# NVIDIA/makani

Measured on NVIDIA H100. Metric: SFNO-block fwd+bwd samples/sec, higher is better.
Workload: dtype tf32

## Files before the change

makani_b200/csrc/dft.cu:

```cuda
#include "umma_common.cuh"
#include "dft_math.cuh"
#include <cmath>
#include <cstdlib>
#include <vector>

namespace b200sht {

int umma_available();

constexpr int kDftMaxHalf = 95;
constexpr int kDftSynWorkers = 10;
constexpr int kDftSynThreads = 32 * (kDftSynWorkers + 2);
constexpr int kDftSynStages = 4;
__host__ __device__ constexpr int dft_out_box(int N2) {
  int d = N2 < 32 ? N2 : 32;
  while (N2 % d != 0) --d;
  return 8 * d;
}

struct DftTables {
  float* et;
  float* eb;
  float2* tw;
  float* zeros;
  int N2, half, M2, nkb;
};

bool dft_shape_ok(int nlon, int mmax) {
  if (nlon % 8 != 0) return false;
  const int N2 = nlon / 8;
  return N2 >= 2 && N2 / 2 <= kDftMaxHalf && (mmax + 7) / 8 <= 32 && mmax <= nlon / 2 + 1;
}

__global__ void dft_tables_kernel(float* et, float* eb, float2* tw, int N2, int half, int M2, int nkb, int nlon) {
  const int i = blockIdx.x * blockDim.x + threadIdx.x;
  if (i < 2 * 128 * 32) {
    const int m2 = i % 32, row = i / 32, p = (row >> 3) & 1, j2 = 8 * (row >> 4) + (row & 7);
    float v = 0.f;
    if (j2 <= half && m2 < M2) {
      const long long t = ((long long)m2 * j2) % N2;
      const double ang = 2.0 * M_PI * (double)t / (double)N2;
      v = tf32_rn((float)(p == 0 ? cos(ang) : sin(ang)));
    }
    et[i] = v;
  }
  if (i < nkb * 2 * 32 * 32) {
    const int jl = i % 32, m2 = (i / 32) % 32, p = (i / 1024) % 2, kb = i / 2048;
    const int j2 = kb * 32 + jl;
    float v = 0.f;
    if (j2 <= half && m2 < M2) {
      const long long t = ((long long)m2 * j2) % N2;
      const double ang = 2.0 * M_PI * (double)t / (double)N2;
      v = tf32_rn((float)(p == 0 ? cos(ang) : sin(ang)));
      if (2 * j2 == N2) v *= 0.5f;
    }
    eb[i] = v;
  }
  if (i < 8 * N2) {
    const int j2 = i % N2, c = i / N2;
    const double ang = 2.0 * M_PI * (double)(c * j2) / (double)nlon;
    tw[i] = make_float2((float)cos(ang), (float)sin(ang));
  }
}

int dft_plan_init(Plan* pl) {
  pl->dft_state = nullptr;
  if (!umma_available()) return -1;
  if (!dft_shape_ok(pl->nlon, pl->mmax)) return -1;
  DftTables* t = new DftTables();
  t->N2 = pl->nlon / 8; t->half = t->N2 / 2; t->M2 = (pl->mmax + 7) / 8;
  t->nkb = (t->half + 1 + 31) / 32;
  t->et = nullptr; t->eb = nullptr; t->tw = nullptr; t->zeros = nullptr;
  const size_t neb = (size_t)t->nkb * 2 * 32 * 32;
  cudaError_t e = cudaMalloc(&t->et, sizeof(float) * 2 * 128 * 32);
  if (e == cudaSuccess) e = cudaMalloc(&t->eb, sizeof(float) * neb);
  if (e == cudaSuccess) e = cudaMalloc(&t->tw, sizeof(float2) * 8 * t->N2);
  if (e == cudaSuccess) e = cudaMalloc(&t->zeros, sizeof(float) * 8 * t->N2);
  if (e == cudaSuccess) e = cudaMemset(t->zeros, 0, sizeof(float) * 8 * t->N2);
  if (e == cudaSuccess) {
    const int n = 8192 > 8 * t->N2 ? 8192 : 8 * t->N2;
    dft_tables_kernel<<<(n + 255) / 256, 256>>>(t->et, t->eb, t->tw, t->N2, t->half, t->M2, t->nkb, pl->nlon);
    e = cudaGetLastError();
    if (e == cudaSuccess) e = cudaStreamSynchronize(0);
  }
  if (e != cudaSuccess) {
    cudaFree(t->et); cudaFree(t->eb); cudaFree(t->tw); cudaFree(t->zeros);
    delete t;
    return -1;
  }
  pl->dft_state = t;
  return 0;
}

void dft_plan_destroy(Plan* pl) {
  DftTables* t = static_cast<DftTables*>(pl->dft_state);
  if (!t) return;
  cudaFree(t->et); cudaFree(t->eb); cudaFree(t->tw); cudaFree(t->zeros);
  delete t;
  pl->dft_state = nullptr;
}

static bool dft_enabled() {
  static const int on = [] { const char* e = getenv("B200SHT_DFT"); return e ? atoi(e) : 1; }();
  return on != 0;
}
bool dft_usable(const Plan* pl) { return pl->dft_state != nullptr && dft_enabled(); }

static unsigned long long* g_dft_prof = nullptr;
static unsigned long long* dft_prof_buffer() {
  static const int on = [] { const char* e = getenv("B200SHT_DFT_PROF"); return e ? atoi(e) : 0; }();
  if (!on) return nullptr;
  if (!g_dft_prof) {
    if (cudaMalloc(&g_dft_prof, 16 * sizeof(unsigned long long)) != cudaSuccess) { g_dft_prof = nullptr; return nullptr; }
    cudaMemset(g_dft_prof, 0, 16 * sizeof(unsigned long long));
  }
  return g_dft_prof;
}
int dft_profile_read(unsigned long long* out16) {
  if (!g_dft_prof) { for (int i = 0; i < 16; ++i) out16[i] = 0; return 0; }
  B200_CHECK_CUDA(cudaDeviceSynchronize());
  B200_CHECK_CUDA(cudaMemcpy(out16, g_dft_prof, 16 * sizeof(unsigned long long), cudaMemcpyDeviceToHost));
  B200_CHECK_CUDA(cudaMemset(g_dft_prof, 0, 16 * sizeof(unsigned long long)));
  return 0;
}
#ifdef B200SHT_DFT_PROFILE
constexpr bool kDftProfile = true;
#else
constexpr bool kDftProfile = false;
#endif
__device__ __forceinline__ void prof_wait(unsigned long long* prof, int slot, uint64_t* bar, uint32_t parity, bool lead) {
  if (!kDftProfile || prof == nullptr) { mbar_wait(bar, parity); return; }
  const long long t0 = clock64();
  mbar_wait(bar, parity);
  if (lead) atomicAdd(prof + slot, (unsigned long long)(clock64() - t0));
}

static int make_tmap_out(CUtensorMap* tm, void* base, bool bf16, int nlon, int nlat, long long rows, int ow) {
  TmapKey key;
  memset(&key, 0, sizeof(key));
  key.base = base; key.rank = 3; key.kind = bf16 ? 7 : 6;
  key.dims[0] = nlon; key.dims[1] = nlat; key.dims[2] = rows; key.box[0] = ow;
  int slot = 0;
  if (tmap_lookup(key, tm, &slot)) return 0;
  PFN_encodeTiled enc = get_encode();
  if (!enc) { set_error("cuTensorMapEncodeTiled is unavailable"); return B200SHT_ERR_UNSUPPORTED; }
  static thread_local bool ctx_bound = false;
  if (!ctx_bound) { cudaFree(nullptr); ctx_bound = true; }
  const int es = bf16 ? 2 : 4;
  cuuint64_t gd[3] = {(cuuint64_t)nlon, (cuuint64_t)nlat, (cuuint64_t)rows};
  cuuint64_t gst[2] = {(cuuint64_t)nlon * es, (cuuint64_t)nlon * nlat * es};
  cuuint32_t bx[3] = {(cuuint32_t)ow, 8, 1}, el[3] = {1, 1, 1};
  if (gst[0] % 16 != 0 || (reinterpret_cast<uintptr_t>(base) & 15) != 0 || (ow * es) % 16 != 0) {
    set_error("tensor map (output): base / row pitch / box row not 16-byte aligned");
    return B200SHT_ERR_INVALID;
  }
  CUresult r = enc(tm, bf16 ? CU_TENSOR_MAP_DATA_TYPE_BFLOAT16 : CU_TENSOR_MAP_DATA_TYPE_FLOAT32, 3, base, gd, gst, bx, el,
                   CU_TENSOR_MAP_INTERLEAVE_NONE, CU_TENSOR_MAP_SWIZZLE_NONE, CU_TENSOR_MAP_L2_PROMOTION_L2_256B, CU_TENSOR_MAP_FLOAT_OOB_FILL_NONE);
  if (r != CUDA_SUCCESS) { set_error("cuTensorMapEncodeTiled (output) failed (%d)", (int)r); return B200SHT_ERR_CUDA; }
  tmap_store(key, tm, slot);
  return 0;
}

template <typename T> __device__ __forceinline__ void st_out(T* p, float v);
template <> __device__ __forceinline__ void st_out<float>(float* p, float v) { *p = v; }
template <> __device__ __forceinline__ void st_out<__nv_bfloat16>(__nv_bfloat16* p, float v) { *p = __float2bfloat16_rn(v); }
template <typename T> __device__ __forceinline__ uint32_t ld_raw(const T* p);
template <> __device__ __forceinline__ uint32_t ld_raw<float>(const float* p) { return __float_as_uint(__ldg(p)); }
template <> __device__ __forceinline__ uint32_t ld_raw<__nv_bfloat16>(const __nv_bfloat16* p) { return (uint32_t)__ldg(reinterpret_cast<const unsigned short*>(p)); }

#ifndef B200_DFT_TF32_MODE
#define B200_DFT_TF32_MODE 2
#endif
constexpr float kTruncComp = 1.0f + 0.0009765625f / 3.0f;
__device__ __forceinline__ float tf32_operand(float v) {
#if B200_DFT_TF32_MODE == 0
  return tf32_rn(v);
#elif B200_DFT_TF32_MODE == 1
  return __uint_as_float((__float_as_uint(v) + 0x1000u) & 0xffffe000u);
#else
  return v;
#endif
}
__device__ __forceinline__ float tf32_operand_unscaled(float v) {
#if B200_DFT_TF32_MODE == 2
  return v * kTruncComp;
#else
  return tf32_operand(v);
#endif
}

__device__ __forceinline__ pr pr_operand(pr v) { return make_pr(tf32_operand(v.v.x), tf32_operand(v.v.y)); }
__device__ __forceinline__ pr pr_operand_unscaled(pr v) {
#if B200_DFT_TF32_MODE == 2
  return rmul(v, kTruncComp);
#else
  return pr_operand(v);
#endif
}

template <typename T> __device__ __forceinline__ float ld_in(const T* p);
template <> __device__ __forceinline__ float ld_in<float>(const float* p) { return __ldg(p); }
template <> __device__ __forceinline__ float ld_in<__nv_bfloat16>(const __nv_bfloat16* p) {
  return __uint_as_float((uint32_t)__ldg(reinterpret_cast<const unsigned short*>(p)) << 16);
}

struct DftSynParams {
  alignas(64) CUtensorMap tmZ;
  alignas(64) CUtensorMap tmE;
  alignas(64) CUtensorMap tmY;
  const float* Z;
  const float2* tw;
  const float* rowscale;
  const float* bias;
  unsigned long long* prof;
  int R, C, nlat, nlon, kp, mmax, N2, half, M2, mode, ntiles, ktiles, has_nyq, ow;
};

template <typename T>
__global__ void __launch_bounds__(kDftSynThreads, 1) dft_synthesis_kernel(const __grid_constant__ DftSynParams p) {
  extern __shared__ uint8_t smem_raw[];
  __shared__ unsigned long long prof_s[16];
  unsigned long long* const prof = (kDftProfile && p.prof) ? prof_s : nullptr;
  if (kDftProfile && threadIdx.x < 16) prof_s[threadIdx.x] = 0;
  const uint32_t raw = smem_u32(smem_raw);
  const uint32_t base = (raw + 1023u) & ~1023u;
  uint8_t* gbase = smem_raw + (base - raw);
  const int N2 = p.N2;
  const int nlon = 8 * N2;
  const int ow = p.ow;
  const uint32_t obytes = (8u * nlon * sizeof(T) + 1023u) & ~1023u;
  const uint32_t sA = base, sB = base + 32768, sO = sB + kDftSynStages * 16384;
  T* const outS = reinterpret_cast<T*>(gbase + (sO - base));
  float2* tws = reinterpret_cast<float2*>(gbase + (sO - base) + 2 * obytes);
  uint64_t* bars = reinterpret_cast<uint64_t*>(reinterpret_cast<uint8_t*>(tws) + ((8 * N2 * 8 + 15) & ~15));
  uint64_t* full = bars;
  uint64_t* empty = full + kDftSynStages;
  uint64_t* e_full = empty + kDftSynStages;
  uint64_t* staged = e_full + 1;
  uint64_t* ofree = staged + 2;

  const int warp = __shfl_sync(0xffffffffu, (int)(threadIdx.x >> 5), 0), lane = threadIdx.x & 31;
  pdl_trigger();
  const int nblk = (p.half + 8) / 8;
  const int nwork = kDftSynWorkers < 2 * nblk ? kDftSynWorkers : 2 * nblk;
  const bool is_tma = (warp == kDftSynWorkers), is_store = (warp == kDftSynWorkers + 1);

  if (threadIdx.x == 0) {
    for (int s = 0; s < kDftSynStages; ++s) { mbar_init(&full[s], 1); mbar_init(&empty[s], nblk); }
    mbar_init(e_full, 1);
    for (int b = 0; b < 2; ++b) { mbar_init(&staged[b], 32 * nblk); mbar_init(&ofree[b], 1); }
    fence_barrier_init();
    prefetch_tmap(&p.tmZ);
    prefetch_tmap(&p.tmE);
    prefetch_tmap(&p.tmY);
  }
  for (int i = threadIdx.x; i < 8 * p.N2; i += blockDim.x) tws[i] = p.tw[i];
  __syncthreads();
  const long long t_cta0 = (kDftProfile && p.prof && threadIdx.x == 0) ? clock64() : 0;
  pdl_wait();

  if (is_tma) {
    if (lane == 0) {
      mbar_expect_tx(e_full, 32768);
      tma_load_2d(sA, &p.tmE, e_full, 0, 0);
      tma_load_2d(sA + 16384, &p.tmE, e_full, 0, 128);
      int n = 0;
      for (int ti = blockIdx.x; ti < p.ntiles; ti += gridDim.x, ++n) {
        const int s = n % kDftSynStages, it = n / kDftSynStages;
        if (it > 0) prof_wait(prof, 8, &empty[s], (it - 1) & 1, true);
        mbar_expect_tx(&full[s], 16384);
        const uint32_t st = sB + s * 16384;
        tma_load_5d(st, &p.tmZ, &full[s], 0, 0, 0, 0, ti);
        tma_load_5d(st + 4096, &p.tmZ, &full[s], 0, 1, 0, 0, ti);
        tma_load_5d(st + 8192, &p.tmZ, &full[s], 0, 0, 0, 1, ti);
        tma_load_5d(st + 12288, &p.tmZ, &full[s], 0, 1, 0, 1, ti);
      }
    }
    __syncwarp();
  } else if (is_store) {
    if (lane == 0) {
      int n = 0;
      for (int ti = blockIdx.x; ti < p.ntiles; ti += gridDim.x, ++n) {
        const int b = n & 1;
        prof_wait(prof, 11, &staged[b], (n >> 1) & 1, true);
        const int r = ti / p.ktiles, k0 = (ti - r * p.ktiles) * 8;
        if (k0 < p.nlat)
          for (int bx = 0; bx * ow < nlon; ++bx) tma_store_3d(&p.tmY, sO + b * obytes + bx * 8 * ow * (uint32_t)sizeof(T), bx * ow, k0, r);
        bulk_commit();
        bulk_wait_read0();
        mbar_arrive(&ofree[b]);
      }
      bulk_wait0();
    }
    __syncwarp();
  } else {
    const int kpi = lane & 3;
    const bool n2odd = (N2 & 1) != 0;
    const float smul = p.mode == 0 ? 2.f : 1.f;
    const int nyq_m = nlon / 2;
    const uint8_t* const gE = gbase;
    mbar_wait(e_full, 0);
    for (int task = warp; warp < nwork; task += nwork) {
      const int n = task / nblk, blk = task - n * nblk;
      const int ti = blockIdx.x + n * gridDim.x;
      if (ti >= p.ntiles) break;
      const int r = ti / p.ktiles, k0 = (ti - r * p.ktiles) * 8;
      const int ka = k0 + 2 * kpi;
      const int s = n % kDftSynStages, it = n / kDftSynStages;
      float rsa = 1.f, rsb = 1.f, z0a = 0.f, z0b = 0.f, zna = 0.f, znb = 0.f;
      if (p.mode == 1) {
        const float2 rs = *reinterpret_cast<const float2*>(p.rowscale + ka);
        rsa = rs.x; rsb = rs.y;
      } else {
        const float* zt = p.Z + (size_t)ti * 2 * p.M2 * 64 + 2 * kpi;
        const float2 z0 = *reinterpret_cast<const float2*>(zt);
        z0a = z0.x; z0b = z0.y;
        if (p.has_nyq) {
          const float2 zn = *reinterpret_cast<const float2*>(zt + (nyq_m >> 3) * 64 + (nyq_m & 7) * 8);
          zna = zn.x; znb = zn.y;
        }
      }
      const float bias = p.bias ? __ldg(p.bias + r % p.C) : 0.f;
      const pr sc = make_pr(smul * rsa, smul * rsb);
      const pr off_e = make_pr(bias - rsa * (z0a + zna), bias - rsb * (z0b + znb));
      const pr off_o = make_pr(bias - rsa * (z0a - zna), bias - rsb * (z0b - znb));
      prof_wait(prof, 9, &full[s], it & 1, lane == 0);
      if (prof && lane == 0) atomicAdd(prof + 13, 1ull);
      float acc[2][8][4];
#pragma unroll
      for (int a = 0; a < 2; ++a)
#pragma unroll
        for (int c = 0; c < 8; ++c) acc[a][c][0] = acc[a][c][1] = acc[a][c][2] = acc[a][c][3] = 0.f;
      {
        const uint8_t* const zs = gbase + 32768 + (size_t)s * 16384;
#pragma unroll
        for (int kk = 0; kk < 32; kk += 8) {
          uint32_t fa[4];
          frag_a<false>(gE, 16 * blk, kk, fa);
#pragma unroll
          for (int c = 0; c < 8; ++c) {
            uint32_t zr[2], zi[2];
            frag_b<true>(zs, 8 * c, kk, zr);
            frag_b<true>(zs + 8192, 8 * c, kk, zi);
            mma_tf32(acc[0][c], fa, zr);
            mma_tf32(acc[1][c], fa, zi);
          }
        }
      }
      __syncwarp();
      if (lane == 0) mbar_arrive(&empty[s]);
      {
        const int j2 = 8 * blk + (lane >> 2);
        const bool valid = j2 <= p.half;
        const bool paired = valid && j2 != 0 && 2 * j2 != N2;
        const int jp = N2 - j2;
        float2 tw[8], tp[8];
        tw[0] = make_float2(1.f, 0.f);
#pragma unroll
        for (int c = 1; c < 8; ++c) tw[c] = valid ? tws[c * N2 + j2] : make_float2(1.f, 0.f);
        dft_partner_twiddles(tw, tp);
        T* const ob = outS + (size_t)(n & 1) * (obytes / sizeof(T)) + 2 * kpi * ow;
        if (n >= 2) prof_wait(prof, 10, &ofree[n & 1], ((n >> 1) - 1) & 1, lane == 0);
        {
          pr vr[8], vi[8], x[8];
#pragma unroll
          for (int c = 0; c < 8; ++c) {
            vr[c] = make_pr(acc[0][c][0], acc[0][c][1]) - make_pr(acc[1][c][2], acc[1][c][3]);
            vi[c] = make_pr(acc[0][c][2], acc[0][c][3]) + make_pr(acc[1][c][0], acc[1][c][1]);
          }
          dft_syn_radix8<pr>(vr, vi, tw, x);
          const pr o0 = (j2 & 1) ? off_o : off_e, o1 = (j2 & 1) ? off_e : off_o;
#pragma unroll
          for (int j1 = 0, bx = j2 / ow, jx = j2 - bx * ow; j1 < 8; ++j1) {
            const pr o = rfma(x[j1], sc, (n2odd && (j1 & 1)) ? o1 : o0);
            if (valid) { st_out<T>(ob + bx * 8 * ow + jx, o.v.x); st_out<T>(ob + bx * 8 * ow + jx + ow, o.v.y); }
            for (jx += N2; jx >= ow; jx -= ow) ++bx;
          }
        }
        {
          pr vr[8], vi[8], x[8];
#pragma unroll
          for (int c = 0; c < 8; ++c) {
            vr[c] = make_pr(acc[0][c][0], acc[0][c][1]) + make_pr(acc[1][c][2], acc[1][c][3]);
            vi[c] = make_pr(acc[1][c][0], acc[1][c][1]) - make_pr(acc[0][c][2], acc[0][c][3]);
          }
          dft_syn_radix8<pr>(vr, vi, tp, x);
          const pr o0 = (jp & 1) ? off_o : off_e, o1 = (jp & 1) ? off_e : off_o;
#pragma unroll
          for (int j1 = 0, bx = jp / ow, jx = jp - bx * ow; j1 < 8; ++j1) {
            const pr o = rfma(x[j1], sc, (n2odd && (j1 & 1)) ? o1 : o0);
            if (paired) { st_out<T>(ob + bx * 8 * ow + jx, o.v.x); st_out<T>(ob + bx * 8 * ow + jx + ow, o.v.y); }
            for (jx += N2; jx >= ow; jx -= ow) ++bx;
          }
        }
        fence_proxy_async();
        mbar_arrive(&staged[n & 1]);
      }
    }
  }
  __syncthreads();
  if (kDftProfile && p.prof && threadIdx.x == 0) prof_s[12] = (unsigned long long)(clock64() - t_cta0);
  if (kDftProfile) __syncthreads();
  if (kDftProfile && p.prof && threadIdx.x < 16) atomicAdd(p.prof + threadIdx.x, prof_s[threadIdx.x]);
}

int dft_synthesis(const Plan* pl, const float* Z, void* y, int dtype, int B, int C, const float* bias, int mode, cudaStream_t st) {
  const DftTables* t = static_cast<const DftTables*>(pl->dft_state);
  B200_REQUIRE(t != nullptr, "dft_synthesis: plan has no DFT tables");
  const int R = B * C;
  DftSynParams p;
  memset(&p, 0, sizeof(p));
  p.Z = Z; p.tw = t->tw; p.rowscale = pl->d_rowscale; p.bias = bias; p.prof = dft_prof_buffer();
  p.R = R; p.C = C; p.nlat = pl->nlat; p.nlon = pl->nlon; p.kp = pl->kp; p.mmax = pl->mmax;
  p.N2 = t->N2; p.half = t->half; p.mode = mode;
  p.ktiles = pl->kp / 8; p.ntiles = R * p.ktiles;
  p.has_nyq = (pl->mmax == pl->nlon / 2 + 1) ? 1 : 0;
  p.M2 = t->M2;
  {
    long long d[5] = {32, 2, t->M2, 2, (long long)R * (pl->kp / 8)}, s[5] = {1, 32, 64, (long long)t->M2 * 64, 2ll * t->M2 * 64};
    int bx[5] = {32, 1, 32, 1, 1};
    int rc = make_tmap(&p.tmZ, Z, 5, d, s, bx);
    if (rc) return rc;
  }
  {
    long long d[2] = {32, 256}, s[2] = {1, 32};
    int bx[2] = {32, 128};
    int rc = make_tmap(&p.tmE, t->et, 2, d, s, bx);
    if (rc) return rc;
  }
  const bool bf16 = (dtype == B200SHT_BF16);
  p.ow = dft_out_box(t->N2);
  {
    int rc = make_tmap_out(&p.tmY, y, bf16, pl->nlon, pl->nlat, R, p.ow);
    if (rc) return rc;
  }
  const size_t obytes = (8 * (size_t)pl->nlon * (bf16 ? 2 : 4) + 1023) & ~(size_t)1023;
  const size_t smem = 1024 + 32768 + (size_t)kDftSynStages * 16384 + 2 * obytes + ((8 * (size_t)t->N2 * 8 + 15) & ~(size_t)15) +
                      (2 * kDftSynStages + 5) * 8;
  const int sms = usable_sms(pl->sm_count > 0 ? pl->sm_count : 132);
  const int ctas = p.ntiles < sms ? p.ntiles : sms;
#define B200_LAUNCH_SYN(TT)                                                                                          \
  do {                                                                                                                \
    struct Tag {};                                                                                                    \
    B200_CHECK_CUDA((ensure_dynamic_smem<Tag>(dft_synthesis_kernel<TT>, smem)));                                     \
    B200_CHECK_CUDA(launch_pdl(dft_synthesis_kernel<TT>, dim3(ctas), dim3(kDftSynThreads), smem, st, p));            \
  } while (0)
  if (bf16) { B200_LAUNCH_SYN(__nv_bfloat16); } else { B200_LAUNCH_SYN(float); }
#undef B200_LAUNCH_SYN
  B200_CHECK_LAUNCH();
  return 0;
}

__host__ __device__ constexpr int dft_box_group(int N2, int es) { return (N2 * es) % 16 == 0 ? 1 : (2 * N2 * es) % 16 == 0 ? 2 : (4 * N2 * es) % 16 == 0 ? 4 : 8; }

static int make_tmap_segments(CUtensorMap* tm, const void* base, bool bf16, int nlon, int gs, long long rows, int box_cols) {
  TmapKey key;
  memset(&key, 0, sizeof(key));
  key.base = base; key.rank = 3; key.kind = bf16 ? 5 : 4;
  key.dims[0] = nlon; key.dims[1] = gs; key.dims[2] = rows; key.box[0] = box_cols;
  int slot = 0;
  if (tmap_lookup(key, tm, &slot)) return 0;
  PFN_encodeTiled enc = get_encode();
  if (!enc) { set_error("cuTensorMapEncodeTiled is unavailable"); return B200SHT_ERR_UNSUPPORTED; }
  static thread_local bool ctx_bound = false;
  if (!ctx_bound) { cudaFree(nullptr); ctx_bound = true; }
  const int es = bf16 ? 2 : 4, N2 = nlon / 8;
  cuuint64_t gd[3] = {(cuuint64_t)gs * N2, (cuuint64_t)(8 / gs), (cuuint64_t)rows};
  cuuint64_t gst[2] = {(cuuint64_t)gs * N2 * es, (cuuint64_t)nlon * es};
  cuuint32_t bx[3] = {(cuuint32_t)box_cols, (cuuint32_t)(8 / gs), 16}, el[3] = {1, 1, 1};
  if (gst[0] % 16 != 0 || gst[1] % 16 != 0 || (reinterpret_cast<uintptr_t>(base) & 15) != 0 || (box_cols * es) % 16 != 0) {
    set_error("tensor map (segments): base / pitch / box row not 16-byte aligned");
    return B200SHT_ERR_INVALID;
  }
  CUresult r = enc(tm, bf16 ? CU_TENSOR_MAP_DATA_TYPE_BFLOAT16 : CU_TENSOR_MAP_DATA_TYPE_FLOAT32, 3, const_cast<void*>(base), gd, gst, bx, el,
                   CU_TENSOR_MAP_INTERLEAVE_NONE, CU_TENSOR_MAP_SWIZZLE_NONE, CU_TENSOR_MAP_L2_PROMOTION_L2_256B, CU_TENSOR_MAP_FLOAT_OOB_FILL_NONE);
  if (r != CUDA_SUCCESS) { set_error("cuTensorMapEncodeTiled (segments) failed (%d)", (int)r); return B200SHT_ERR_CUDA; }
  tmap_store(key, tm, slot);
  return 0;
}

constexpr int kDftAnaStages = 2;
constexpr int kDftAnaMma = 8, kDftAnaLoader = 8, kDftAnaProd0 = 9, kDftAnaThreads = 512;

struct DftAnaParams {
  alignas(64) CUtensorMap tmB;
  alignas(64) CUtensorMap tmXc;
  alignas(64) CUtensorMap tmXp;
  float* X;
  const float2* tw;
  const float* rowscale;
  unsigned long long* prof;
  int R, nlat, nlon, kp, mmax, N2, half, M2, nkb, mode, ntiles, ktiles, nraw, gs;
};

template <typename T, int N2T>
__global__ void __launch_bounds__(kDftAnaThreads, 1) dft_analysis_kernel(const __grid_constant__ DftAnaParams p) {
  extern __shared__ uint8_t smem_raw[];
  __shared__ unsigned long long prof_s[16];
  unsigned long long* const prof = (kDftProfile && p.prof) ? prof_s : nullptr;
  if (kDftProfile && threadIdx.x < 16) prof_s[threadIdx.x] = 0;
  const uint32_t raw = smem_u32(smem_raw);
  const uint32_t base = (raw + 1023u) & ~1023u;
  uint8_t* gbase = smem_raw + (base - raw);
  constexpr int kAl = 16 / (int)sizeof(T);
  constexpr int kWc = (sizeof(T) == 2) ? 40 : 32, kWp = (sizeof(T) == 2) ? 40 : 36;
  constexpr uint32_t kColBytes = 16u * kWc * sizeof(T), kParBytes = 16u * kWp * sizeof(T);
  constexpr uint32_t kRawBytes = 8u * (kColBytes + kParBytes);
  const uint32_t oB = 0, oA = 3 * 8192, oR = oA + kDftAnaStages * 65536, oT = oR + (uint32_t)p.nraw * kRawBytes, oBar = oT + 3 * 7 * 32 * 8;
  const uint32_t sBm = base + oB, sAr = base + oA, sRaw = base + oR;
  uint8_t* gA = gbase + oA;
  const uint8_t* gR = gbase + oR;
  float2* twS = reinterpret_cast<float2*>(gbase + oT);
  uint64_t* full = reinterpret_cast<uint64_t*>(gbase + oBar);
  uint64_t* empty = full + kDftAnaStages;
  uint64_t* raw_full = empty + kDftAnaStages;
  uint64_t* raw_empty = raw_full + 4;
  uint64_t* b_full = raw_empty + 4;

  const int warp = __shfl_sync(0xffffffffu, (int)(threadIdx.x >> 5), 0), lane = threadIdx.x & 31;
  pdl_trigger();
  const int nkb = p.nkb;
  const int N2 = N2T > 0 ? N2T : p.N2;
  const int gs = N2T > 0 ? dft_box_group(N2T, (int)sizeof(T)) : p.gs;
  for (int i = threadIdx.x; i < nkb * 7 * 32; i += blockDim.x) {
    const int ln = i & 31, c = (i >> 5) % 7 + 1, kb = i / 224;
    const int j2 = 32 * kb + ln;
    float2 w = (j2 <= p.half) ? p.tw[c * N2 + j2] : make_float2(1.f, 0.f);
#if B200_DFT_TF32_MODE == 2
    w.x *= kTruncComp; w.y *= kTruncComp;
#endif
    twS[i] = w;
  }
  if (threadIdx.x == 0) {
    for (int s = 0; s < kDftAnaStages; ++s) { mbar_init(&full[s], 8); mbar_init(&empty[s], kDftAnaMma); }
    for (int s = 0; s < p.nraw; ++s) { mbar_init(&raw_full[s], 1); mbar_init(&raw_empty[s], 8); }
    mbar_init(b_full, 1);
    fence_barrier_init();
    prefetch_tmap(&p.tmB);
    prefetch_tmap(&p.tmXc);
    prefetch_tmap(&p.tmXp);
  }
  for (int i = threadIdx.x; i < kDftAnaStages * 2 * 512; i += blockDim.x) {
    const int st = i >> 10, pl = (i >> 9) & 1, off = i & 511;
    reinterpret_cast<float*>(gA + (size_t)st * 65536)[(pl ? 12288 : 4096) + off] = 0.f;
  }
  __syncthreads();
  const long long t_cta0 = (kDftProfile && p.prof && threadIdx.x == 0) ? clock64() : 0;
  pdl_wait();

  if (warp == kDftAnaLoader) {
    if (lane == 0) {
      mbar_expect_tx(b_full, (uint32_t)nkb * 8192);
      for (int kb = 0; kb < nkb; ++kb) {
        tma_load_2d(sBm + kb * 8192, &p.tmB, b_full, 0, kb * 64);
        tma_load_2d(sBm + kb * 8192 + 4096, &p.tmB, b_full, 0, kb * 64 + 32);
      }
      int n = 0;
      for (int ti = blockIdx.x; ti < p.ntiles; ti += gridDim.x, ++n) {
        const int r = ti / p.ktiles, row0 = r * p.nlat + (ti - r * p.ktiles) * 16;
        for (int kb = 0; kb < nkb; ++kb) {
          const int g = n * nkb + kb, rs = g % p.nraw, it = g / p.nraw;
          if (it > 0) prof_wait(prof, 2, &raw_empty[rs], (it - 1) & 1, true);
          mbar_expect_tx(&raw_full[rs], kRawBytes);
          const uint32_t dst = sRaw + rs * kRawBytes;
#pragma unroll
          for (int gm = 0; gm < 8; ++gm) {
            if (gm >= gs) break;
            const int sc = N2 * gm + 32 * kb, sp = N2 * gm + N2 - 32 * kb - 31;
            tma_load_3d(dst + gm * (8 / gs) * kColBytes, &p.tmXc, &raw_full[rs], (sc / kAl) * kAl, 0, row0);
            tma_load_3d(dst + 8 * kColBytes + gm * (8 / gs) * kParBytes, &p.tmXp, &raw_full[rs], sp < 0 ? 0 : (sp / kAl) * kAl, 0, row0);
          }
        }
      }
    }
    __syncwarp();
  } else if (warp < kDftAnaMma) {
    const size_t plane = (size_t)p.R * p.kp;
    const int c = warp, gq = lane >> 2, q = lane & 3;
    mbar_wait(b_full, 0);
    int n = 0;
    for (int ti = blockIdx.x; ti < p.ntiles; ti += gridDim.x, ++n) {
      const int r = ti / p.ktiles, k0 = (ti - r * p.ktiles) * 16;
      float xr[4][4], xi[4][4];
#pragma unroll
      for (int j = 0; j < 4; ++j)
#pragma unroll
        for (int e = 0; e < 4; ++e) { xr[j][e] = 0.f; xi[j][e] = 0.f; }
      for (int kb = 0; kb < nkb; ++kb) {
        const int g = n * nkb + kb, s = g % kDftAnaStages, it = g / kDftAnaStages;
        prof_wait(prof, 3, &full[s], it & 1, lane == 0);
        const uint8_t* const a0 = gA + (size_t)s * 65536;
        const uint8_t* const bc = gbase + oB + kb * 8192;
#pragma unroll
        for (int half = 0; half < 2; ++half) {
          const uint32_t col = 32 * q + 16 * half;
          uint4 av[4][2];
#pragma unroll
          for (int pl = 0; pl < 4; ++pl)
#pragma unroll
            for (int h = 0; h < 2; ++h) av[pl][h] = lds128(a0 + pl * 16384, (16 * c + gq + 8 * h) * 128 + col);
#pragma unroll
          for (int cs = 0; cs < 2; ++cs) {
            uint4 bv[4];
#pragma unroll
            for (int j = 0; j < 4; ++j) bv[j] = lds128(bc + cs * 4096, (8 * j + gq) * 128 + col);
            const int pr_ = cs ? 3 : 0, pi_ = cs ? 2 : 1;
#pragma unroll
            for (int t = 0; t < 2; ++t) {
              uint32_t far_[4], fai[4];
              far_[0] = t ? av[pr_][0].z : av[pr_][0].x; far_[1] = t ? av[pr_][1].z : av[pr_][1].x;
              far_[2] = t ? av[pr_][0].w : av[pr_][0].y; far_[3] = t ? av[pr_][1].w : av[pr_][1].y;
              fai[0] = t ? av[pi_][0].z : av[pi_][0].x; fai[1] = t ? av[pi_][1].z : av[pi_][1].x;
              fai[2] = t ? av[pi_][0].w : av[pi_][0].y; fai[3] = t ? av[pi_][1].w : av[pi_][1].y;
              if (cs) frag_neg(fai, fai);
#pragma unroll
              for (int j = 0; j < 4; ++j) {
                const uint32_t fb[2] = {t ? bv[j].z : bv[j].x, t ? bv[j].w : bv[j].y};
                mma_tf32(xr[j], far_, fb);
                mma_tf32(xi[j], fai, fb);
              }
            }
          }
        }
        __syncwarp();
        if (lane == 0) mbar_arrive(&empty[s]);
      }
      if (prof && lane == 0) atomicAdd(prof + 5, 1ull);
#pragma unroll
      for (int h = 0; h < 2; ++h) {
        const int k = k0 + gq + 8 * h;
        if (k >= p.kp) continue;
        const float rs = (p.mode == 0) ? ((k < p.nlat) ? __ldg(p.rowscale + k) : 0.f) : 1.f;
        float* xb = p.X + (size_t)r * p.kp + k;
#pragma unroll
        for (int j = 0; j < 4; ++j)
#pragma unroll
          for (int e = 0; e < 2; ++e) {
            const int m = c + 8 * (8 * j + 2 * q + e);
            if (m >= p.mmax) continue;
            const float sc = ((p.mode == 0) ? rs : ((m == 0 || 2 * m == p.nlon) ? 1.f : 2.f)) * kTruncComp;
            float* dst = xb + (size_t)m * 2 * plane;
            dst[0] = __uint_as_float(__float_as_uint(xr[j][2 * h + e] * sc) & 0xffffe000u);
            dst[plane] = __uint_as_float(__float_as_uint(xi[j][2 * h + e] * sc) & 0xffffe000u);
          }
      }
    }
  } else {
    const int pw = warp - kDftAnaProd0;
    constexpr int nprod = kDftAnaThreads / 32 - kDftAnaProd0;
    static_assert(nprod >= 1 && nprod <= 8, "every producer warp must take an item of every K-block (8 items each)");
    constexpr bool kBf16 = (sizeof(T) == 2);
    const T* const rawS = reinterpret_cast<const T*>(gR);
    int n = 0;
    for (int ti = blockIdx.x; ti < p.ntiles; ti += gridDim.x, ++n) {
      const int r = ti / p.ktiles, kt16 = (ti - r * p.ktiles) * 16;
      for (int item = pw; item < 8 * nkb; item += nprod) {
        const int kb = item >> 3, q = item & 7;
        const int k0 = kt16 + 2 * q;
        const int g = n * nkb + kb;
        const int j2 = 32 * kb + lane;
        const int rs = g % p.nraw;
        prof_wait(prof, 0, &raw_full[rs], (g / p.nraw) & 1, lane == 0);
        if (prof && lane == 0) atomicAdd(prof + 7, 1ull);
        const T* const rb = rawS + (size_t)rs * (kRawBytes / sizeof(T));
        pr xa[8], xb[8];
#pragma unroll
        for (int j1 = 0; j1 < 8; ++j1) {
          const int gm = j1 % gs, ga = j1 / gs, npb = 8 / gs;
          const int sc = N2 * gm + 32 * kb, sp = N2 * gm + N2 - 32 * kb - 31;
          const int ic = sc - (sc / kAl) * kAl + lane;
          int ip = N2 * gm + N2 - j2 - (sp < 0 ? 0 : (sp / kAl) * kAl);
          ip = ip < 0 ? 0 : (ip > kWp - 1 ? kWp - 1 : ip);
          const T* b0 = rb + gm * (16 * npb * kWc) + (2 * q) * (npb * kWc) + ga * kWc;
          const T* b1 = rb + 8 * (16 * kWc) + gm * (16 * npb * kWp) + (2 * q) * (npb * kWp) + ga * kWp;
          const int rowc = npb * kWc, rowp = npb * kWp;
          if constexpr (kBf16) {
            xa[j1] = make_pr(__uint_as_float((uint32_t)reinterpret_cast<const unsigned short*>(b0)[ic] << 16),
                             __uint_as_float((uint32_t)reinterpret_cast<const unsigned short*>(b0)[rowc + ic] << 16));
            xb[j1] = make_pr(__uint_as_float((uint32_t)reinterpret_cast<const unsigned short*>(b1)[ip] << 16),
                             __uint_as_float((uint32_t)reinterpret_cast<const unsigned short*>(b1)[rowp + ip] << 16));
          } else {
            xa[j1] = make_pr(reinterpret_cast<const float*>(b0)[ic], reinterpret_cast<const float*>(b0)[rowc + ic]);
            xb[j1] = make_pr(reinterpret_cast<const float*>(b1)[ip], reinterpret_cast<const float*>(b1)[rowp + ip]);
          }
        }
        __syncwarp();
        if (lane == 0) mbar_arrive(&raw_empty[rs]);
        if (kb == 0) {
#pragma unroll
          for (int j1 = 0; j1 < 8; ++j1) xb[j1] = (lane == 0) ? make_pr(0.f, 0.f) : xb[j1];
        }
        if (k0 + 1 >= p.nlat) {
          const bool row0ok = k0 < p.nlat;
#pragma unroll
          for (int j1 = 0; j1 < 8; ++j1) {
            xa[j1] = make_pr(row0ok ? xa[j1].v.x : 0.f, 0.f);
            xb[j1] = make_pr(row0ok ? xb[j1].v.x : 0.f, 0.f);
          }
        }
        pr er[8], ei[8], br[8], bi[8];
        float2 tw[8], tp[8];
        tw[0] = make_float2(1.f, 0.f);
        const float2* const twl = twS + kb * 224 + lane;
#pragma unroll
        for (int c = 1; c < 8; ++c) tw[c] = twl[(c - 1) * 32];
        dft_partner_twiddles(tw, tp);
        dft_ana_radix8<pr>(xa, tw, er, ei);
        dft_ana_radix8<pr>(xb, tp, br, bi);
        const int s = g % kDftAnaStages, it = g / kDftAnaStages;
        if (it > 0) prof_wait(prof, 1, &empty[s], (it - 1) & 1, lane == 0);
        float* const stg = reinterpret_cast<float*>(gA + (size_t)s * 65536);
        const int kr0 = 2 * q;
        float* const d0 = stg + kr0 * 32 + ((((lane >> 2) ^ (kr0 & 7)) << 2) | (lane & 3));
        float* const d1 = stg + (kr0 + 1) * 32 + ((((lane >> 2) ^ ((kr0 + 1) & 7)) << 2) | (lane & 3));
#pragma unroll
        for (int c = 0; c < 8; ++c) {
          pr ye_r = er[c] + br[c], yo_r = er[c] - br[c];
          if (c == 0) { ye_r = pr_operand_unscaled(ye_r); yo_r = pr_operand_unscaled(yo_r); }
          else { ye_r = pr_operand(ye_r); yo_r = pr_operand(yo_r); }
          d0[c * 512] = ye_r.v.x; d1[c * 512] = ye_r.v.y;
          d0[8192 + c * 512] = yo_r.v.x; d1[8192 + c * 512] = yo_r.v.y;
          if (c != 0) {
            const pr ye_i = pr_operand(ei[c] + bi[c]), yo_i = pr_operand(ei[c] - bi[c]);
            d0[4096 + c * 512] = ye_i.v.x; d1[4096 + c * 512] = ye_i.v.y;
            d0[12288 + c * 512] = yo_i.v.x; d1[12288 + c * 512] = yo_i.v.y;
          }
        }
        fence_proxy_async();
        __syncwarp();
        if (lane == 0) mbar_arrive(&full[s]);
      }
    }
  }
  __syncthreads();
  if (kDftProfile && p.prof && threadIdx.x == 0) prof_s[6] = (unsigned long long)(clock64() - t_cta0);
  if (kDftProfile) __syncthreads();
  if (kDftProfile && p.prof && threadIdx.x < 16) atomicAdd(p.prof + threadIdx.x, prof_s[threadIdx.x]);
}

int dft_analysis(const Plan* pl, const void* x, int dtype, int B, int C, float* X, int mode, cudaStream_t st) {
  const DftTables* t = static_cast<const DftTables*>(pl->dft_state);
  B200_REQUIRE(t != nullptr, "dft_analysis: plan has no DFT tables");
  const int R = B * C;
  DftAnaParams p;
  memset(&p, 0, sizeof(p));
  p.X = X; p.tw = t->tw; p.rowscale = pl->d_rowscale; p.prof = dft_prof_buffer();
  p.R = R; p.nlat = pl->nlat; p.nlon = pl->nlon; p.kp = pl->kp; p.mmax = pl->mmax;
  p.N2 = t->N2; p.half = t->half; p.M2 = t->M2; p.nkb = t->nkb; p.mode = mode;
  p.ktiles = (pl->kp + 15) / 16; p.ntiles = R * p.ktiles;
  const bool bf16 = (dtype == B200SHT_BF16);
  p.nraw = bf16 ? 3 : 2;
  {
    long long d[2] = {32, (long long)t->nkb * 64}, s[2] = {1, 32};
    int bx[2] = {32, 32};
    int rc = make_tmap(&p.tmB, t->eb, 2, d, s, bx);
    if (rc) return rc;
  }
  B200_REQUIRE(bf16 || t->N2 % 4 == 0, "dft_analysis: fp32 input needs nlon %% 32 == 0 (16-byte aligned TMA boxes)");
  {
    p.gs = dft_box_group(t->N2, bf16 ? 2 : 4);
    int rc = make_tmap_segments(&p.tmXc, x, bf16, pl->nlon, p.gs, (long long)R * pl->nlat, bf16 ? 40 : 32);
    if (!rc) rc = make_tmap_segments(&p.tmXp, x, bf16, pl->nlon, p.gs, (long long)R * pl->nlat, bf16 ? 40 : 36);
    if (rc) return rc;
  }
  const size_t raw_bytes = bf16 ? (size_t)8 * 16 * (40 + 40) * 2 : (size_t)8 * 16 * (32 + 36) * 4;
  const size_t smem = 1024 + 3 * 8192 + (size_t)kDftAnaStages * 65536 + p.nraw * raw_bytes + 3 * 7 * 32 * 8 + 256;
  const int sms = usable_sms(pl->sm_count > 0 ? pl->sm_count : 132);
  const int ctas = p.ntiles < sms ? p.ntiles : sms;
  const int threads = kDftAnaThreads;
#define B200_LAUNCH_ANA(TT, NN)                                                                                                          \
  do {                                                                                                                                  \
    struct Tag {};                                                                                                                        \
    B200_CHECK_CUDA((ensure_dynamic_smem<Tag>(dft_analysis_kernel<TT, NN>, smem)));                                                      \
    B200_CHECK_CUDA(launch_pdl(dft_analysis_kernel<TT, NN>, dim3(ctas), dim3(threads), smem, st, p));                                                                         \
  } while (0)
#define B200_DISPATCH_ANA(TT)                                            \
  switch (t->N2) {                                                       \
    case 180: B200_LAUNCH_ANA(TT, 180); break;            \
    case 90: B200_LAUNCH_ANA(TT, 90); break;              \
    case 60: B200_LAUNCH_ANA(TT, 60); break;              \
    default: B200_LAUNCH_ANA(TT, 0); break;                              \
  }
  if (bf16) { B200_DISPATCH_ANA(__nv_bfloat16) } else { B200_DISPATCH_ANA(float) }
#undef B200_DISPATCH_ANA
#undef B200_LAUNCH_ANA
  B200_CHECK_LAUNCH();
  return 0;
}

int dft_host(int N, int mmax, int direction, int mode, const float* rowscale, const float* in, float* out) {
  if (!dft_shape_ok(N, mmax)) { set_error("debug_dft_host: unsupported (nlon=%d, mmax=%d)", N, mmax); return B200SHT_ERR_UNSUPPORTED; }
  const int N2 = N / 8, half = N2 / 2, M2 = (mmax + 7) / 8;
  const float rs = rowscale ? rowscale[0] : 1.f;
  auto twid = [&](int j, float2* tw) {
    for (int c = 0; c < 8; ++c) {
      const double a = 2.0 * M_PI * (double)(c * j) / (double)N;
      tw[c] = make_float2((float)cos(a), (float)sin(a));
    }
  };
  if (direction == 1) {
    std::vector<double> zr(8 * M2, 0.0), zi(8 * M2, 0.0);
    for (int m = 0; m < mmax; ++m) { zr[m] = in[2 * m]; zi[m] = in[2 * m + 1]; }
    const bool has_nyq = (mmax == N / 2 + 1);
    for (int j2 = 0; j2 <= half; ++j2) {
      float s1[8], s2[8], s3[8], s4[8];
      for (int c = 0; c < 8; ++c) {
        double a1 = 0, a2 = 0, a3 = 0, a4 = 0;
        for (int m2 = 0; m2 < M2; ++m2) {
          const double b = 2.0 * M_PI * (double)(((long long)m2 * j2) % N2) / (double)N2;
          a1 += cos(b) * zr[c + 8 * m2]; a2 += sin(b) * zi[c + 8 * m2]; a3 += sin(b) * zr[c + 8 * m2]; a4 += cos(b) * zi[c + 8 * m2];
        }
        s1[c] = (float)a1; s2[c] = (float)a2; s3[c] = (float)a3; s4[c] = (float)a4;
      }
      float2 tw[8], tp[8];
      twid(j2, tw);
      dft_partner_twiddles(tw, tp);
      for (int side = 0; side < 2; ++side) {
        if (side == 1 && (j2 == 0 || 2 * j2 == N2)) continue;
        const int jj = side ? N2 - j2 : j2;
        float vr[8], vi[8], x[8];
        for (int c = 0; c < 8; ++c) {
          vr[c] = side ? s1[c] + s2[c] : s1[c] - s2[c];
          vi[c] = side ? s4[c] - s3[c] : s3[c] + s4[c];
        }
        dft_syn_radix8<float>(vr, vi, side ? tp : tw, x);
        for (int j1 = 0; j1 < 8; ++j1) {
          const int j = N2 * j1 + jj;
          float v = x[j1];
          if (mode == 0) {
            v = 2.f * v - (float)zr[0];
            if (has_nyq) v -= (float)zr[N / 2] * ((j & 1) ? -1.f : 1.f);
          } else {
            v *= rs;
          }
          out[j] = v;
        }
      }
    }
    return 0;
  }
  std::vector<double> dre(8 * M2, 0.0), dim(8 * M2, 0.0);
  for (int j2 = 0; j2 <= half; ++j2) {
    float2 tw[8], tp[8];
    twid(j2, tw);
    dft_partner_twiddles(tw, tp);
    float xa[8], er[8], ei[8], orr[8], oi[8];
    for (int j1 = 0; j1 < 8; ++j1) xa[j1] = in[N2 * j1 + j2];
    dft_ana_radix8<float>(xa, tw, er, ei);
    const bool paired = (j2 != 0 && 2 * j2 != N2);
    if (paired) {
      float xb[8], br[8], bi[8];
      for (int j1 = 0; j1 < 8; ++j1) xb[j1] = in[N2 * j1 + N2 - j2];
      dft_ana_radix8<float>(xb, tp, br, bi);
      for (int c = 0; c < 8; ++c) { orr[c] = er[c] - br[c]; oi[c] = ei[c] - bi[c]; er[c] += br[c]; ei[c] += bi[c]; }
    } else {
      for (int c = 0; c < 8; ++c) { orr[c] = 0.f; oi[c] = 0.f; }
    }
    for (int c = 0; c < 8; ++c)
      for (int m2 = 0; m2 < M2; ++m2) {
        const double b = 2.0 * M_PI * (double)(((long long)m2 * j2) % N2) / (double)N2;
        dre[c + 8 * m2] += cos(b) * er[c] + sin(b) * oi[c];
        dim[c + 8 * m2] += cos(b) * ei[c] - sin(b) * orr[c];
      }
  }
  for (int m = 0; m < mmax; ++m) {
    const double sc = mode == 0 ? (double)rs : ((m == 0 || 2 * m == N) ? 1.0 : 2.0);
    out[2 * m] = (float)(dre[m] * sc);
    out[2 * m + 1] = (float)(dim[m] * sc);
  }
  return 0;
}

}
```

Before: 756.6.

## Use WGMMA for DFT analysis GEMM and precompute synthesis output offsets

Replaces the per-warp mma.sync TF32 loop in the DFT analysis kernel with warpgroup wgmma using shared-memory descriptors. Accumulators stay asynchronous with one group in flight, and the empty-barrier release is deferred by one stage. The synthesis kernel now precomputes output scatter offsets in a shared table and uses a precomputed swizzle offset for the B fragment loads. Barrier waits switch to a non-call variant, and the full barrier now counts every thread's arrival. The analysis kernel's thread count also changes to 544, and whether that matches the warpgroup layout assumptions is risky.

```diff
diff --git a/makani_b200/csrc/dft.cu b/makani_b200/csrc/dft.cu
--- a/makani_b200/csrc/dft.cu
+++ b/makani_b200/csrc/dft.cu
@@ -1,4 +1,5 @@
 #include "umma_common.cuh"
+#include "wgmma_tf32.cuh"
 #include "dft_math.cuh"
 #include <cmath>
 #include <cstdlib>
@@ -134,6 +135,12 @@
   mbar_wait(bar, parity);
   if (lead) atomicAdd(prof + slot, (unsigned long long)(clock64() - t0));
 }
+__device__ __forceinline__ void prof_wait_nocall(unsigned long long* prof, int slot, uint64_t* bar, uint32_t parity, bool lead) {
+  if (!kDftProfile || prof == nullptr) { mbar_wait_nocall(bar, parity); return; }
+  const long long t0 = clock64();
+  mbar_wait_nocall(bar, parity);
+  if (lead) atomicAdd(prof + slot, (unsigned long long)(clock64() - t0));
+}
 
 static int make_tmap_out(CUtensorMap* tm, void* base, bool bf16, int nlon, int nlat, long long rows, int ow) {
   TmapKey key;
@@ -232,7 +239,8 @@
   const uint32_t sA = base, sB = base + 32768, sO = sB + kDftSynStages * 16384;
   T* const outS = reinterpret_cast<T*>(gbase + (sO - base));
   float2* tws = reinterpret_cast<float2*>(gbase + (sO - base) + 2 * obytes);
-  uint64_t* bars = reinterpret_cast<uint64_t*>(reinterpret_cast<uint8_t*>(tws) + ((8 * N2 * 8 + 15) & ~15));
+  int* oofs = reinterpret_cast<int*>(reinterpret_cast<uint8_t*>(tws) + ((8 * N2 * 8 + 15) & ~15));
+  uint64_t* bars = reinterpret_cast<uint64_t*>(reinterpret_cast<uint8_t*>(oofs) + 8 * N2 * 4);
   uint64_t* full = bars;
   uint64_t* empty = full + kDftSynStages;
   uint64_t* e_full = empty + kDftSynStages;
@@ -255,6 +263,10 @@
     prefetch_tmap(&p.tmY);
   }
   for (int i = threadIdx.x; i < 8 * p.N2; i += blockDim.x) tws[i] = p.tw[i];
+  for (int i = threadIdx.x; i < 8 * N2; i += blockDim.x) {
+    const int j = N2 * (i & 7) + (i >> 3);
+    oofs[i] = (j / ow) * 8 * ow + j % ow;
+  }
   __syncthreads();
   const long long t_cta0 = (kDftProfile && p.prof && threadIdx.x == 0) ? clock64() : 0;
   pdl_wait();
@@ -299,6 +311,11 @@
     const float smul = p.mode == 0 ? 2.f : 1.f;
     const int nyq_m = nlon / 2;
     const uint8_t* const gE = gbase;
+    uint32_t zoff[2][4];
+#pragma unroll
+    for (int h = 0; h < 2; ++h)
+#pragma unroll
+      for (int cc = 0; cc < 4; ++cc) zoff[h][cc] = swz128((uint32_t)((kpi + 4 * h) * 128 + (8 * cc + (lane >> 2)) * 4));
     mbar_wait(e_full, 0);
     for (int task = warp; warp < nwork; task += nwork) {
       const int n = task / nblk, blk = task - n * nblk;
@@ -339,9 +356,10 @@
           frag_a<false>(gE, 16 * blk, kk, fa);
 #pragma unroll
           for (int c = 0; c < 8; ++c) {
-            uint32_t zr[2], zi[2];
-            frag_b<true>(zs, 8 * c, kk, zr);
-            frag_b<true>(zs + 8192, 8 * c, kk, zi);
+            const uint8_t* const zc = zs + (c >> 2) * 4096 + kk * 128;
+            const uint32_t zr[2] = {*reinterpret_cast<const uint32_t*>(zc + zoff[0][c & 3]), *reinterpret_cast<const uint32_t*>(zc + zoff[1][c & 3])};
+            const uint32_t zi[2] = {*reinterpret_cast<const uint32_t*>(zc + 8192 + zoff[0][c & 3]),
+                                    *reinterpret_cast<const uint32_t*>(zc + 8192 + zoff[1][c & 3])};
             mma_tf32(acc[0][c], fa, zr);
             mma_tf32(acc[1][c], fa, zi);
           }
@@ -370,11 +388,13 @@
           }
           dft_syn_radix8<pr>(vr, vi, tw, x);
           const pr o0 = (j2 & 1) ? off_o : off_e, o1 = (j2 & 1) ? off_e : off_o;
-#pragma unroll
-          for (int j1 = 0, bx = j2 / ow, jx = j2 - bx * ow; j1 < 8; ++j1) {
+          const int4* const op = reinterpret_cast<const int4*>(oofs + 8 * (valid ? j2 : 0));
+          const int4 oa = op[0], ob4 = op[1];
+          const int of[8] = {oa.x, oa.y, oa.z, oa.w, ob4.x, ob4.y, ob4.z, ob4.w};
+#pragma unroll
+          for (int j1 = 0; j1 < 8; ++j1) {
             const pr o = rfma(x[j1], sc, (n2odd && (j1 & 1)) ? o1 : o0);
-            if (valid) { st_out<T>(ob + bx * 8 * ow + jx, o.v.x); st_out<T>(ob + bx * 8 * ow + jx + ow, o.v.y); }
-            for (jx += N2; jx >= ow; jx -= ow) ++bx;
+            if (valid) { st_out<T>(ob + of[j1], o.v.x); st_out<T>(ob + of[j1] + ow, o.v.y); }
           }
         }
         {
@@ -386,11 +406,13 @@
           }
           dft_syn_radix8<pr>(vr, vi, tp, x);
           const pr o0 = (jp & 1) ? off_o : off_e, o1 = (jp & 1) ? off_e : off_o;
-#pragma unroll
-          for (int j1 = 0, bx = jp / ow, jx = jp - bx * ow; j1 < 8; ++j1) {
+          const int4* const op = reinterpret_cast<const int4*>(oofs + 8 * (paired ? jp : 0));
+          const int4 oa = op[0], ob4 = op[1];
+          const int of[8] = {oa.x, oa.y, oa.z, oa.w, ob4.x, ob4.y, ob4.z, ob4.w};
+#pragma unroll
+          for (int j1 = 0; j1 < 8; ++j1) {
             const pr o = rfma(x[j1], sc, (n2odd && (j1 & 1)) ? o1 : o0);
-            if (paired) { st_out<T>(ob + bx * 8 * ow + jx, o.v.x); st_out<T>(ob + bx * 8 * ow + jx + ow, o.v.y); }
-            for (jx += N2; jx >= ow; jx -= ow) ++bx;
+            if (paired) { st_out<T>(ob + of[j1], o.v.x); st_out<T>(ob + of[j1] + ow, o.v.y); }
           }
         }
         fence_proxy_async();
@@ -436,7 +458,7 @@
   }
   const size_t obytes = (8 * (size_t)pl->nlon * (bf16 ? 2 : 4) + 1023) & ~(size_t)1023;
   const size_t smem = 1024 + 32768 + (size_t)kDftSynStages * 16384 + 2 * obytes + ((8 * (size_t)t->N2 * 8 + 15) & ~(size_t)15) +
-                      (2 * kDftSynStages + 5) * 8;
+                      8 * (size_t)t->N2 * 4 + (2 * kDftSynStages + 5) * 8;
   const int sms = usable_sms(pl->sm_count > 0 ? pl->sm_count : 132);
   const int ctas = p.ntiles < sms ? p.ntiles : sms;
 #define B200_LAUNCH_SYN(TT)                                                                                          \
@@ -480,7 +502,7 @@
 }
 
 constexpr int kDftAnaStages = 2;
-constexpr int kDftAnaMma = 8, kDftAnaLoader = 8, kDftAnaProd0 = 9, kDftAnaThreads = 512;
+constexpr int kDftAnaMma = 8, kDftAnaLoader = 8, kDftAnaProd0 = 9, kDftAnaThreads = 544;
 
 struct DftAnaParams {
   alignas(64) CUtensorMap tmB;
@@ -532,7 +554,7 @@
     twS[i] = w;
   }
   if (threadIdx.x == 0) {
-    for (int s = 0; s < kDftAnaStages; ++s) { mbar_init(&full[s], 8); mbar_init(&empty[s], kDftAnaMma); }
+    for (int s = 0; s < kDftAnaStages; ++s) { mbar_init(&full[s], 8 * 32); mbar_init(&empty[s], kDftAnaMma); }
     for (int s = 0; s < p.nraw; ++s) { mbar_init(&raw_full[s], 1); mbar_init(&raw_empty[s], 8); }
     mbar_init(b_full, 1);
     fence_barrier_init();
@@ -544,6 +566,7 @@
     const int st = i >> 10, pl = (i >> 9) & 1, off = i & 511;
     reinterpret_cast<float*>(gA + (size_t)st * 65536)[(pl ? 12288 : 4096) + off] = 0.f;
   }
+  fence_proxy_async();
   __syncthreads();
   const long long t_cta0 = (kDftProfile && p.prof && threadIdx.x == 0) ? clock64() : 0;
   pdl_wait();
@@ -560,7 +583,7 @@
         const int r = ti / p.ktiles, row0 = r * p.nlat + (ti - r * p.ktiles) * 16;
         for (int kb = 0; kb < nkb; ++kb) {
           const int g = n * nkb + kb, rs = g % p.nraw, it = g / p.nraw;
-          if (it > 0) prof_wait(prof, 2, &raw_empty[rs], (it - 1) & 1, true);
+          if (it > 0) prof_wait_nocall(prof, 2, &raw_empty[rs], (it - 1) & 1, true);
           mbar_expect_tx(&raw_full[rs], kRawBytes);
           const uint32_t dst = sRaw + rs * kRawBytes;
 #pragma unroll
@@ -577,54 +600,37 @@
   } else if (warp < kDftAnaMma) {
     const size_t plane = (size_t)p.R * p.kp;
     const int c = warp, gq = lane >> 2, q = lane & 3;
-    mbar_wait(b_full, 0);
+    const uint32_t aw = sAr + (uint32_t)(warp >> 2) * 8192;
+    mbar_wait_nocall(b_full, 0);
     int n = 0;
     for (int ti = blockIdx.x; ti < p.ntiles; ti += gridDim.x, ++n) {
       const int r = ti / p.ktiles, k0 = (ti - r * p.ktiles) * 16;
-      float xr[4][4], xi[4][4];
-#pragma unroll
-      for (int j = 0; j < 4; ++j)
-#pragma unroll
-        for (int e = 0; e < 4; ++e) { xr[j][e] = 0.f; xi[j][e] = 0.f; }
+      float acc[8][4];
+      int prev = 0;
       for (int kb = 0; kb < nkb; ++kb) {
         const int g = n * nkb + kb, s = g % kDftAnaStages, it = g / kDftAnaStages;
-        prof_wait(prof, 3, &full[s], it & 1, lane == 0);
-        const uint8_t* const a0 = gA + (size_t)s * 65536;
-        const uint8_t* const bc = gbase + oB + kb * 8192;
-#pragma unroll
-        for (int half = 0; half < 2; ++half) {
-          const uint32_t col = 32 * q + 16 * half;
-          uint4 av[4][2];
-#pragma unroll
-          for (int pl = 0; pl < 4; ++pl)
-#pragma unroll
-            for (int h = 0; h < 2; ++h) av[pl][h] = lds128(a0 + pl * 16384, (16 * c + gq + 8 * h) * 128 + col);
-#pragma unroll
-          for (int cs = 0; cs < 2; ++cs) {
-            uint4 bv[4];
-#pragma unroll
-            for (int j = 0; j < 4; ++j) bv[j] = lds128(bc + cs * 4096, (8 * j + gq) * 128 + col);
-            const int pr_ = cs ? 3 : 0, pi_ = cs ? 2 : 1;
-#pragma unroll
-            for (int t = 0; t < 2; ++t) {
-              uint32_t far_[4], fai[4];
-              far_[0] = t ? av[pr_][0].z : av[pr_][0].x; far_[1] = t ? av[pr_][1].z : av[pr_][1].x;
-              far_[2] = t ? av[pr_][0].w : av[pr_][0].y; far_[3] = t ? av[pr_][1].w : av[pr_][1].y;
-              fai[0] = t ? av[pi_][0].z : av[pi_][0].x; fai[1] = t ? av[pi_][1].z : av[pi_][1].x;
-              fai[2] = t ? av[pi_][0].w : av[pi_][0].y; fai[3] = t ? av[pi_][1].w : av[pi_][1].y;
-              if (cs) frag_neg(fai, fai);
-#pragma unroll
-              for (int j = 0; j < 4; ++j) {
-                const uint32_t fb[2] = {t ? bv[j].z : bv[j].x, t ? bv[j].w : bv[j].y};
-                mma_tf32(xr[j], far_, fb);
-                mma_tf32(xi[j], fai, fb);
-              }
-            }
-          }
-        }
-        __syncwarp();
-        if (lane == 0) mbar_arrive(&empty[s]);
-      }
+        prof_wait_nocall(prof, 3, &full[s], it & 1, lane == 0);
+        const uint32_t a0 = aw + (uint32_t)s * 65536;
+        const uint64_t d_er = wgmma_desc_kmajor(a0), d_ei = wgmma_desc_kmajor(a0 + 16384);
+        const uint64_t d_or = wgmma_desc_kmajor(a0 + 32768), d_oi = wgmma_desc_kmajor(a0 + 49152);
+        const uint64_t d_c = wgmma_desc_kmajor(sBm + kb * 8192), d_s = wgmma_desc_kmajor(sBm + kb * 8192 + 4096);
+        wgmma_fence();
+#pragma unroll
+        for (int k = 0; k < 4; ++k) {
+          const int sd = (kb > 0 || k > 0) ? 1 : 0;
+          wgmma_tf32<32, 1, 8, 0>(acc, d_er + 2 * k, d_c + 2 * k, sd);
+          wgmma_tf32<32, 1, 8, 4>(acc, d_ei + 2 * k, d_c + 2 * k, sd);
+          wgmma_tf32<32, 1, 8, 0>(acc, d_oi + 2 * k, d_s + 2 * k, 1);
+          wgmma_tf32<32, -1, 8, 4>(acc, d_or + 2 * k, d_s + 2 * k, 1);
+        }
+        wgmma_commit();
+        wgmma_wait<1>();
+        if (kb > 0 && lane == 0) mbar_arrive(&empty[prev]);
+        prev = s;
+      }
+      wgmma_wait<0>();
+      wgmma_fence_operands(acc);
+      if (lane == 0) mbar_arrive(&empty[prev]);
       if (prof && lane == 0) atomicAdd(prof + 5, 1ull);
 #pragma unroll
       for (int h = 0; h < 2; ++h) {
@@ -640,8 +646,8 @@
             if (m >= p.mmax) continue;
             const float sc = ((p.mode == 0) ? rs : ((m == 0 || 2 * m == p.nlon) ? 1.f : 2.f)) * kTruncComp;
             float* dst = xb + (size_t)m * 2 * plane;
-            dst[0] = __uint_as_float(__float_as_uint(xr[j][2 * h + e] * sc) & 0xffffe000u);
-            dst[plane] = __uint_as_float(__float_as_uint(xi[j][2 * h + e] * sc) & 0xffffe000u);
+            dst[0] = __uint_as_float(__float_as_uint(acc[j][2 * h + e] * sc) & 0xffffe000u);
+            dst[plane] = __uint_as_float(__float_as_uint(acc[4 + j][2 * h + e] * sc) & 0xffffe000u);
           }
       }
     }
@@ -660,7 +666,7 @@
         const int g = n * nkb + kb;
         const int j2 = 32 * kb + lane;
         const int rs = g % p.nraw;
-        prof_wait(prof, 0, &raw_full[rs], (g / p.nraw) & 1, lane == 0);
+        prof_wait_nocall(prof, 0, &raw_full[rs], (g / p.nraw) & 1, lane == 0);
         if (prof && lane == 0) atomicAdd(prof + 7, 1ull);
         const T* const rb = rawS + (size_t)rs * (kRawBytes / sizeof(T));
         pr xa[8], xb[8];
@@ -684,8 +690,6 @@
             xb[j1] = make_pr(reinterpret_cast<const float*>(b1)[ip], reinterpret_cast<const float*>(b1)[rowp + ip]);
           }
         }
-        __syncwarp();
-        if (lane == 0) mbar_arrive(&raw_empty[rs]);
         if (kb == 0) {
 #pragma unroll
           for (int j1 = 0; j1 < 8; ++j1) xb[j1] = (lane == 0) ? make_pr(0.f, 0.f) : xb[j1];
@@ -707,8 +711,10 @@
         dft_partner_twiddles(tw, tp);
         dft_ana_radix8<pr>(xa, tw, er, ei);
         dft_ana_radix8<pr>(xb, tp, br, bi);
+        __syncwarp();
+        if (lane == 0) mbar_arrive(&raw_empty[rs]);
         const int s = g % kDftAnaStages, it = g / kDftAnaStages;
-        if (it > 0) prof_wait(prof, 1, &empty[s], (it - 1) & 1, lane == 0);
+        if (it > 0) prof_wait_nocall(prof, 1, &empty[s], (it - 1) & 1, lane == 0);
         float* const stg = reinterpret_cast<float*>(gA + (size_t)s * 65536);
         const int kr0 = 2 * q;
         float* const d0 = stg + kr0 * 32 + ((((lane >> 2) ^ (kr0 & 7)) << 2) | (lane & 3));
@@ -727,8 +733,7 @@
           }
         }
         fence_proxy_async();
-        __syncwarp();
-        if (lane == 0) mbar_arrive(&full[s]);
+        mbar_arrive(&full[s]);
       }
     }
   }
```

After: 855.1, median of 6. 1.13x the previous value.
